# wangjunchi/LLMSeg

Measured on AMD Instinct MI355X. Metric: images/sec (1024x1024, 64-tok prompt) model_forward fwd+bwd, higher is better.
Workload: dtype bf16; 1 GPU; BASELINE.json configs[2]: synthetic 1024x1024 + random-init LLaVA-7B(Llama-7B+CLIP-L/14)/SAM-ViT-H, batch_size=2 per GPU, fwd+bwd train step (CE + align + IoP losses, LoRA r=8 dropout 0.05 on q/v + trainable embed/lm_head/text_fcs/lisa_*, frozen towers, fp32 gradient arena, AdamW step every 10 micro-steps inside the timed region, micro-step replayed from a hipGraph), 256 candidate masks, 64-token ; global_batch=2, parallelism=dp1, graph=True, valid=True

## Files before the change

### llmseg_amd/csrc/capi.cpp

```cpp
#include <hip/hip_runtime.h>
#include <stdarg.h>
#include <stdio.h>
#include <stdlib.h>
#include <algorithm>
#include <array>
#include <map>
#include <mutex>
#include <string>
#include <vector>
#include "llmseg_hip.h"

static thread_local char g_err[512] = "";

void llmseg_set_error(const char* fmt, ...) {
  va_list ap;
  va_start(ap, fmt);
  vsnprintf(g_err, sizeof(g_err), fmt, ap);
  va_end(ap);
}

extern "C" const char* llmseg_last_error(void) { return g_err; }

#include <atomic>
static std::atomic<long> g_launches{0};
// ... 53 lines not shown
  g_prof_on = on != 0;
  return LLMSEG_OK;
}

extern "C" const char* llmseg_prof_dominant_kernel(void) { return g_dom_name; }
extern "C" double llmseg_prof_dominant_bytes(void) { return g_dom_bytes; }
extern "C" int llmseg_prof_dominant_info(int64_t* out4) {
  if (!out4) return LLMSEG_EINVAL;
  for (int i = 0; i < 4; ++i) out4[i] = g_dom_info[i];
  return LLMSEG_OK;
}

extern "C" int llmseg_prof_collect(double* total_ms, double* total_flops, int64_t* launches, double* dom_ms, double* dom_flops, int64_t* dom_launches) {
  std::lock_guard<std::mutex> lk(g_mu);
  double ms = 0, fl = 0;
  std::map<long, std::array<double, 4>> by_class;
  std::map<std::array<long, 4>, std::array<double, 3>> by_shape;
  std::map<long, std::array<int64_t, 3>> split_by_class;
  for (auto& r : g_recs) {
    (void)hipEventSynchronize(r.b);
    float t = 0;
    (void)hipEventElapsedTime(&t, r.a, r.b);
    ms += t;
    fl += r.flops;
    auto& c = by_class[((r.tag[3] % 10000) / 1000) * 2 + (r.tag[3] & 1)];
    c[0] += t; c[1] += r.flops; c[2] += 1;
    {
      const long S = r.tag[3] / 10000;
      auto& sp = split_by_class[((r.tag[3] % 10000) / 1000) * 2 + (r.tag[3] & 1)];
      if (S > 1) { sp[0] += 1; sp[1] += S; }
    }
    c[3] += 2.0 * ((double)r.tag[0] * r.tag[2] + (double)r.tag[1] * r.tag[2] + (double)r.tag[0] * r.tag[1]);
    auto& e = by_shape[{r.tag[0], r.tag[1], r.tag[2], r.tag[3]}];
    e[0] += t; e[1] += r.flops; e[2] += 1;
    g_pool.push_back(r);
  }
  if (getenv("LLMSEG_PROF_TABLE")) {
    std::vector<std::pair<double, std::array<long, 4>>> order;
    for (auto& kv : by_shape) order.push_back({-kv.second[0], kv.first});
    std::sort(order.begin(), order.end());
    fprintf(stderr, "%8s %8s %8s %6s %8s %10s %9s %6s\n", "M", "N", "K", "var", "calls", "total_ms", "TFLOP/s", "%time");
    const size_t top = (size_t)std::max(40, atoi(getenv("LLMSEG_PROF_TABLE")));
    for (size_t i = 0; i < order.size() && i < top; ++i) {
      auto& e = by_shape[order[i].second];
      fprintf(stderr, "%8ld %8ld %8ld %6ld %8.0f %10.2f %9.1f %6.1f\n", order[i].second[0], order[i].second[1], order[i].second[2], order[i].second[3],
              e[2], e[0], e[1] / (e[0] * 1e-3) / 1e12, 100.0 * e[0] / ms);
    }
  }
  if (total_ms) *total_ms = ms;
  if (total_flops) *total_flops = fl;
  if (launches) *launches = (int64_t)g_recs.size();
  long dom = -1;
  for (auto& kv : by_class) if (dom < 0 || kv.second[0] > by_class[dom][0]) dom = kv.first;
  static const char* names[] = {"gemm_bf16_tn_kernel<*, ...> (register staging, 128x128)", "?", "gemm_bf16_tn_glds_kernel<*, 2, 1>", "gemm_skinny_kernel<M>", "?", "?", "?", "gemm_bf16_tn_pp2_kernel<*, false>",
                                "gemm_bf16_tn_pp_kernel<*, false, 4>", "gemm_bf16_tn_pp_kernel<*, false, 2>"};
  if (dom >= 0) {
    const long v = dom / 2;
    std::string nm = (v >= 0 && v < 10) ? names[v] : "?";
    const size_t star = nm.find('*');
    if (star != std::string::npos) nm.replace(star, 1, (dom & 1) ? "true" : "false");
    snprintf(g_dom_name, sizeof(g_dom_name), "%s", nm.c_str());
  } else g_dom_name[0] = 0;
  if (dom_ms) *dom_ms = dom >= 0 ? by_class[dom][0] : 0;
  if (dom_flops) *dom_flops = dom >= 0 ? by_class[dom][1] : 0;
  if (dom_launches) *dom_launches = dom >= 0 ? (int64_t)by_class[dom][2] : 0;
  g_dom_bytes = dom >= 0 ? by_class[dom][3] : 0;
  if (dom >= 0) {
    const auto& sp = split_by_class[dom];
    g_dom_info[0] = (int64_t)by_class[dom][2]; g_dom_info[1] = sp[0]; g_dom_info[2] = sp[1]; g_dom_info[3] = (int64_t)by_class[dom][2] + sp[0];
  } else g_dom_info[0] = g_dom_info[1] = g_dom_info[2] = g_dom_info[3] = 0;
  g_recs.clear();
  return LLMSEG_OK;
}
```

### llmseg_amd/csrc/gemm.hip

```cpp
#include <algorithm>
#include <cstdlib>
#include "common.h"
#include "llmseg_hip.h"

namespace {

constexpr int BN = 128, BK = 64, NT = 256;
constexpr int GROUP_M = 8;

struct GemmP {
  const bf16_t* A; const bf16_t* W; void* C;
  const bf16_t* bias; const bf16_t* gamma; const bf16_t* res;
  int M, N, K;
  long lda, ldw, ldc, ldr, sA, sW, sC, sA2, sW2, sC2;
  int batch1;
  float alpha;
  int act;
  int tiles_m, tiles_n;
  int c_vec, r_vec, b_vec;
  const bf16_t* A2; const bf16_t* W2; long lda2, ldw2;
  int group_m;
  int skew;
  int kt_total;
  int accum;
// ... 897 lines not shown
  const int nt = nt_main + (EXT ? 1 : 0);
  auto ext_a = [&](int h, int i) {
    const int ra = PP_AROW0(h, i) + (lane >> 3);
    return p.A2 + (long)min(m0 + ra, p.M - 1) * p.lda2 + (((lane & 7) ^ ((ra >> 1) & 7)) << 3);
  };
  auto ext_w = [&](int h, int i) {
    const int rw = PP_WROW0(h, i) + (lane >> 3);
    return p.W2 + (long)min(n0 + rw, p.N - 1) * p.ldw2 + (((lane & 7) ^ ((rw >> 1) & 7)) << 3);
  };

  f32x4_t acc[4][2 * MI];
#pragma unroll
  for (int nb = 0; nb < 4; ++nb)
#pragma unroll
    for (int mb = 0; mb < 2 * MI; ++mb) acc[nb][mb] = f32x4_t{0.f, 0.f, 0.f, 0.f};
  bf16x8_t af[MI][2], wf0[2][2], wf1[2][2];
  const int frow = lane & 15, fq = lane >> 4;
  const int wrow0 = FX == FX_ROPE ? (wn >> 1) * 128 + (wn & 1) * 32 : FX == FX_SWIGLU ? wn * 32 : wn * 64;
  const int wrow1 = wrow0 + (FX == FX_ROPE ? 64 : FX == FX_SWIGLU ? 128 : 32);

  char* cur = smem;
  char* nxt = smem + BUF;
  char* nn = smem + 2 * BUF;
  if (EXT) { PP_ISSUE_AX(0, cur); PP_ISSUE_WX(0, cur); PP_ISSUE_WX(1, cur); PP_ISSUE_AX(1, cur); }
  else { PP_ISSUE_A(0, 0, cur); PP_ISSUE_W(0, 0, cur); PP_ISSUE_W(1, 0, cur); PP_ISSUE_A(1, 0, cur); }
  PP_ISSUE_A(0, 1, nxt); PP_ISSUE_W(0, 1, nxt); PP_ISSUE_W(1, 1, nxt); PP_ISSUE_A(1, 1, nxt);
  PP_VMI(6);
  __builtin_amdgcn_s_barrier();
  if (wm == 1) __builtin_amdgcn_s_barrier();
  __builtin_amdgcn_sched_barrier(0);

#define PP2_READ_A P16_READ_W(wf0, 0, cur); P16_READ_W(wf1, 1, cur); P16_READ_A(0, cur)
#define PP2_MMA_A P16_MMA(wf0, 0, 0); P16_MMA(wf1, 2, 0)
#define PP2_MMA_B P16_MMA(wf1, 2, MI); P16_MMA(wf0, 0, MI)
  int t = 0;
  for (; t < nt - 2; ++t) {
    PP_PHASE(PP2_READ_A, PP_ISSUE_A(0, t + 2, nn); PP_ISSUE_W(0, t + 2, nn), PP_NOP, PP2_MMA_A);
    PP_PHASE(P16_READ_A(MI, cur), PP_ISSUE_W(1, t + 2, nn); PP_ISSUE_A(1, t + 2, nn), PP_VMI(6), PP2_MMA_B);
    char* const tmp = cur; cur = nxt; nxt = nn; nn = tmp;
  }
  PP_PHASE(PP2_READ_A, PP_NOP, PP_NOP, PP2_MMA_A);
  PP_PHASE(P16_READ_A(MI, cur), PP_NOP, PP_VM_0, PP2_MMA_B);
  cur = nxt;
  PP_PHASE(PP2_READ_A, PP_NOP, PP_NOP, PP2_MMA_A);
  PP_PHASE(P16_READ_A(MI, cur), PP_NOP, PP_NOP, PP2_MMA_B);
#undef PP2_READ_A
#undef PP2_MMA_A
#undef PP2_MMA_B
  if (wm == 0) __builtin_amdgcn_s_barrier();
  if constexpr (FX != FX_NONE) epilogue_fx<MI, FX>(p, Acc16<MI>{acc}, smem, wave, m0, n0, wm, wn, lane);
  else epilogue_lds<OUT_F32, MI>(p, Acc16<MI>{acc}, smem, wave, m0, n0, wm, wn, lane, bz);
}

template <int MT, int AT, bool SK = false>
__global__ __launch_bounds__(256) void gemm_skinny_kernel(GemmP p, int out_f32) {
  constexpr int KS = MT >= 4 ? 1 : 2;
  constexpr int STEP = KS * 512;
  constexpr int ADV = SK ? 4 * STEP : STEP;
  constexpr int XB = AT == 2 ? MT : 1;
  const int lane = threadIdx.x & 63, wave = threadIdx.x >> 6;
  const int n0 = SK ? blockIdx.x * 4 : (blockIdx.x * 4 + wave) * 4;
  if (n0 >= p.N) return;
  const bf16_t* wr[4];
#pragma unroll
  for (int r = 0; r < 4; ++r) wr[r] = p.W + (long)min(n0 + r, p.N - 1) * p.ldw;
  float acc[4][MT];
#pragma unroll
  for (int r = 0; r < 4; ++r)
#pragma unroll
    for (int m = 0; m < MT; ++m) acc[r][m] = 0.f;
  const int K = p.K;
  auto loadw = [&](uint4 (&w)[KS][4], int k) {
#pragma unroll
    for (int t = 0; t < KS; ++t)
#pragma unroll
      for (int r = 0; r < 4; ++r) w[t][r] = *reinterpret_cast<const uint4*>(wr[r] + min(k + t * 512, K - 8));
  };
  auto loadx = [&](uint4 (&xa)[KS][MT], uint4 (&xb)[KS][XB], int k) {
#pragma unroll
    for (int t = 0; t < KS; ++t) {
      const int kk = k + t * 512, kc = min(kk, K - 8);
      const bool ok = kk < K;
#pragma unroll
      for (int m = 0; m < MT; ++m) {
        const bf16_t* ar = p.A + (long)min(m, p.M - 1) * p.lda;
        const uint4 v = *reinterpret_cast<const uint4*>(ar + kc);
        xa[t][m] = make_uint4(ok ? v.x : 0u, ok ? v.y : 0u, ok ? v.z : 0u, ok ? v.w : 0u);
        if constexpr (AT == 2) xb[t][m] = *reinterpret_cast<const uint4*>(ar + K + kc);
      }
      if constexpr (AT == 1) xb[t][0] = *reinterpret_cast<const uint4*>(p.a_norm_w + kc);
    }
  };
  float rstd[MT];
  auto xform = [&](const uint4& a, const uint4& b, int m) -> uint4 {
    if constexpr (AT == 0) return a;
    float f[8], g[8], o[8];
    unpack8(a, f);
    unpack8(b, g);
    if constexpr (AT == 1) {
      const float r = rstd[m];
      const uint4 xn = make_uint4(pack2bf(f[0] * r, f[1] * r), pack2bf(f[2] * r, f[3] * r), pack2bf(f[4] * r, f[5] * r), pack2bf(f[6] * r, f[7] * r));
      unpack8(xn, f);
#pragma unroll
      for (int e = 0; e < 8; ++e) o[e] = g[e] * f[e];
    } else {
#pragma unroll
// ... 211 lines not shown
__global__ __launch_bounds__(256) void splitk_reduce_delta_kernel(GemmP p, const float* __restrict__ slab, int S, const bf16_t* __restrict__ O, long ldo,
                                                                 float* __restrict__ delta, int heads, int T) {
  const long m = blockIdx.x;
  const int nch = p.N >> 3;
  const long slab_sz = (long)p.M * p.N;
  const long b = m / T, q = m - b * T;
#pragma unroll
  for (int i = 0; i < CPT; ++i) {
    const int c = threadIdx.x + 256 * i;
    if (c < nch) {
      const int n = c * 8;
      const float* sp = slab + m * p.N + n;
      float4 a0 = *reinterpret_cast<const float4*>(sp), a1 = *reinterpret_cast<const float4*>(sp + 4);
      for (int s2 = 1; s2 < S; ++s2) {
        const float4 b0 = *reinterpret_cast<const float4*>(sp + s2 * slab_sz), b1 = *reinterpret_cast<const float4*>(sp + s2 * slab_sz + 4);
        a0.x += b0.x; a0.y += b0.y; a0.z += b0.z; a0.w += b0.w;
        a1.x += b1.x; a1.y += b1.y; a1.z += b1.z; a1.w += b1.w;
      }
      const float v[8] = {a0.x * p.alpha, a0.y * p.alpha, a0.z * p.alpha, a0.w * p.alpha, a1.x * p.alpha, a1.y * p.alpha, a1.z * p.alpha, a1.w * p.alpha};
      const uint4 g = pack8(v);
      *reinterpret_cast<uint4*>(reinterpret_cast<bf16_t*>(p.C) + m * p.ldc + n) = g;
      float of[8], df[8];
      unpack8(*reinterpret_cast<const uint4*>(O + m * ldo + n), of);
      unpack8(g, df);
      float part = 0.f;
#pragma unroll
      for (int e = 0; e < 8; ++e) part = fmaf(of[e], df[e], part);
#pragma unroll
      for (int mm = 8; mm >= 1; mm >>= 1) part += __shfl_xor(part, mm, 64);
      if ((c & 15) == 0) delta[(b * heads + (c >> 4)) * T + q] = part;
    }
  }
}

struct NormReq { const bf16_t* w; bf16_t* out; long ldn; float eps; bool active, done; };
static thread_local NormReq g_norm_req = {nullptr, nullptr, 0, 0.f, false, false};
struct NbReq { const llmseg_gemm_args* a; void* out; bool active, done; };
static thread_local NbReq g_nb_req = {nullptr, nullptr, false, false};
struct DlReq { const llmseg_gemm_args* a; bool active, done; };
static thread_local DlReq g_dl_req = {nullptr, false, false};

template <bool OUT_F32, int MI, int NBUF>
void launch_glds(const GemmP& p, dim3 grid, hipStream_t s) {
  LL_LAUNCH_KERNEL((gemm_bf16_tn_glds_kernel<OUT_F32, MI, NBUF>), grid, dim3(NT), 0, s, p);
}

}

void llmseg_prof_begin(hipStream_t s);
void llmseg_prof_end(hipStream_t s, double flops);
void llmseg_prof_tag(long a, long b, long c, long d);

static int g_gemm_variant = 5, g_gemm_skew = 13, g_gemm_split = 0, g_gemm_pp2 = getenv("LLMSEG_GEMM_PP2") ? atoi(getenv("LLMSEG_GEMM_PP2")) : 1;
static const int g_gemm_rsplit = getenv("LLMSEG_GEMM_NO_RSPLIT") ? 0 : 1;
static int num_cus() {
  static int n = [] { int dev = 0, v = 0; (void)hipGetDevice(&dev); (void)hipDeviceGetAttribute(&v, hipDeviceAttributeMultiprocessorCount, dev); return v > 0 ? v : 256; }();
  return n;
}
extern "C" int llmseg_gemm_set_variant(int v) {
  g_gemm_variant = v & 15;
  if ((v >> 4) & 15) g_gemm_skew = ((v >> 4) & 15) - 1;
  g_gemm_split = (v >> 8) & 31;
  g_gemm_pp2 = (v >> 13) & 3 ? ((v >> 13) & 3) - 1 : g_gemm_pp2;
  return LLMSEG_OK;
}

namespace {
struct GemmPlan { int variant, split; double us; };
inline double pp_cost(long M, long N, int nt, int mi, int S, long ncu, bool f32out) {
  const long tiles = ((M + 64 * mi - 1) / (64 * mi)) * ((N + 255) / 256);
  const long rounds = (tiles * S + ncu - 1) / ncu;
  const int q = (nt + S - 1) / S;
  const double it = mi == 4 ? 1.7 : 1.0, fix = (mi == 4 ? 7.0 : 4.5) + ((S > 1 || f32out) ? 1.0 : 0.0);
  double eff_rounds = (double)rounds;
  if (S == 1) {
    const long full = tiles / ncu, rem = tiles - full * ncu;
    eff_rounds = (double)full + (rem ? 0.5 + 0.5 * (double)rem / (double)ncu : 0.0);
  }
  double us = eff_rounds * (q * it + fix);
  if (S > 1) us += 2.5 + ((double)(S + 1) * M * N * 4.0) / 4.0e6;
  return us;
}
inline double glds_cost(long M, long N, int nt, long ncu) {
  const long tiles = ((M + 127) / 128) * ((N + 127) / 128);
  const long full = tiles / (4 * ncu), rem = tiles - full * 4 * ncu;
  double us = (double)full * (nt * 2.4 + 4.0);
  if (rem > 0) { const double w = (double)((rem + ncu - 1) / ncu); us += nt * std::max(1.3, 0.6 * w) + 4.0; }
  return us;
}
inline bool split_ok(int nt, int S) {
  if (S <= 1) return S == 1;
  const int q = (nt + S - 1) / S;
  return q >= 2 && nt - (S - 1) * q >= 2;
}
}

static int gemm_dispatch(const llmseg_gemm_args* a, void* stream, int force_variant);

extern "C" int llmseg_norm(const void* x, const void* w, const void* b, void* y, int64_t rows, int64_t cols, int64_t ldx, int64_t ldy, float eps, int rms,
                           const int32_t* row_map, void* stream);

extern "C" int llmseg_rope(void* x, const float* cos, const float* sin, int64_t rows, int64_t T, int32_t heads, int32_t head_dim, int64_t ld, void* stream);
extern "C" int llmseg_swiglu(const void* gu, void* out, int64_t rows, int64_t I, int64_t ldgu, int64_t ldo, void* stream);
extern "C" __attribute__((visibility("hidden"))) int llmseg_swiglu_bwd_ld(const void* gu, const void* dout, void* dgu, int64_t rows, int64_t I, int64_t ld_dout, void* stream);

static thread_local bool g_fx_done = false;
static const bool g_fx_off = getenv("LLMSEG_GEMM_NO_FX") != nullptr;

static int gemm_fx(const llmseg_gemm_args* a, void* stream) {
  LL_CHECK(a->fx >= 1 && a->fx <= 3, "gemm: unknown fx %d", a->fx);
  LL_CHECK(!a->out_f32 && a->batch <= 1 && a->batch2 <= 1 && a->alpha == 1.f && !a->bias && !a->gamma && !a->residual && a->act == LLMSEG_ACT_NONE && !a->norm_out &&
               !a->trans_a && !a->trans_w && !a->accumulate, "gemm: fx needs a plain bf16 product (batch 1, alpha 1, no bias / activation / gamma / residual / norm_out)");
  if (a->fx == LLMSEG_FX_ROPE) {
    LL_CHECK(a->fx_cos && a->fx_sin && a->fx_T > 0 && a->fx_cols > 0 && (a->fx_cols % 128) == 0 && a->fx_cols <= a->N && (a->ldc & 3) == 0 &&
                 ((((uintptr_t)a->fx_cos) | ((uintptr_t)a->fx_sin)) & 15) == 0 && (((uintptr_t)a->C) & 7) == 0,
             "gemm: fx rope needs fp32 [fx_T][64] tables (16-byte aligned), fx_cols a multiple of 128 (heads of width 128) and <= N");
  } else if (a->fx == LLMSEG_FX_SWIGLU) {
    LL_CHECK(a->fx_out && (a->N & 15) == 0 && (a->fx_ld & 7) == 0 && a->fx_ld >= a->N / 2 && (a->ldc & 7) == 0 && !a->A2 && ((((uintptr_t)a->fx_out) | ((uintptr_t)a->C)) & 15) == 0,
             "gemm: fx swiglu needs N = 2 I with I %% 8 == 0, fx_out bf16 [M][fx_ld >= I], 16-byte aligned rows, no extension operands");
  } else {
    LL_CHECK(a->fx_in && (a->N & 7) == 0 && (a->fx_ld & 7) == 0 && a->fx_ld >= 2 * a->N && a->ldc >= 2 * a->N && (a->ldc & 7) == 0 && !a->A2 &&
                 ((((uintptr_t)a->fx_in) | ((uintptr_t)a->C)) & 15) == 0,
             "gemm: fx swiglu_bwd needs N = I, fx_in = gate|up bf16 [M][fx_ld >= 2 I], C = d(gate|up) [M][ldc >= 2 I], 16-byte aligned rows");
  }
  g_fx_done = false;
  llmseg_gemm_args g = *a;
// ... 74 lines not shown
  if (a && a->struct_size == sizeof(*a) && a->dl_o) return gemm_dl(a, stream);
  if (!(a && a->struct_size == sizeof(*a) && a->norm_out)) return gemm_dispatch(a, stream, -1);
  LL_CHECK(a->norm_w && !a->out_f32 && a->batch <= 1 && a->batch2 <= 1 && (a->N & 7) == 0 && (a->ldn & 7) == 0 && a->ldn >= a->N && (a->ldc & 7) == 0 &&
               ((((uintptr_t)a->norm_w) | ((uintptr_t)a->norm_out) | ((uintptr_t)a->C)) & 15) == 0 && !a->accumulate,
           "gemm: norm_out needs norm_w, bf16 output, batch 1, N, ldc and ldn multiples of 8, 16-byte aligned pointers");
  g_norm_req = NormReq{(const bf16_t*)a->norm_w, (bf16_t*)a->norm_out, (long)a->ldn, a->norm_eps, true, false};
  const int rc = gemm_dispatch(a, stream, -1);
  const bool done = g_norm_req.done;
  g_norm_req.active = false;
  if (rc != LLMSEG_OK || done) return rc;
  return llmseg_norm(a->C, a->norm_w, nullptr, a->norm_out, a->M, a->N, a->ldc, a->ldn, a->norm_eps, 1, nullptr, stream);
}

static int gemm_dispatch(const llmseg_gemm_args* a, void* stream, int force_variant) {
  LL_CHECK(a && a->struct_size == sizeof(*a), "%s: ABI mismatch: caller's struct_size %u != %zu (bind against include/llmseg_hip.h version %d)",
           "gemm", a ? a->struct_size : 0u, sizeof(*a), LLMSEG_ABI_VERSION);
  LL_CHECK(a && a->A && a->W && a->C, "gemm: null pointer");
  LL_CHECK(a->M > 0 && a->N > 0 && a->K > 0, "gemm: bad shape M=%ld N=%ld K=%ld", (long)a->M, (long)a->N, (long)a->K);
  const bool ta = a->trans_a != 0, tw = a->trans_w != 0;
  LL_CHECK((a->lda & 7) == 0 && (a->ldw & 7) == 0, "gemm: lda/ldw must be multiples of 8 (lda=%ld ldw=%ld)", (long)a->lda, (long)a->ldw);
  const long k8 = (a->K + 7) & ~7L;
  LL_CHECK((ta || (a->K & 7) == 0 || a->lda >= k8) && (tw || (a->K & 7) == 0 || a->ldw >= k8),
           "gemm: K=%ld is not a multiple of 8 and the K-contiguous operand is not padded", (long)a->K);
  LL_CHECK((!ta || a->lda >= a->M) && (!tw || a->ldw >= a->N), "gemm: transposed operand needs ld >= rows");
  LL_CHECK((((uintptr_t)a->A) & 15) == 0 && (((uintptr_t)a->W) & 15) == 0, "gemm: A/W must be 16-byte aligned");
  LL_CHECK(((a->strideA | a->strideW | a->strideA2 | a->strideW2) & 7) == 0, "gemm: batch strides of A/W must be multiples of 8");
  LL_CHECK(!a->accumulate || a->out_f32, "gemm: accumulate needs fp32 output");
  const int esz = a->out_f32 ? 4 : 2;
  GemmP p;
  p.A = (const bf16_t*)a->A; p.W = (const bf16_t*)a->W; p.C = a->C;
  p.bias = (const bf16_t*)a->bias; p.gamma = (const bf16_t*)a->gamma; p.res = (const bf16_t*)a->residual;
  p.M = (int)a->M; p.N = (int)a->N; p.K = (int)a->K;
  p.lda = a->lda; p.ldw = a->ldw; p.ldc = a->ldc; p.ldr = a->residual ? a->ldr : 0;
  const long batch1 = a->batch > 0 ? a->batch : 1, batch2 = a->batch2 > 0 ? a->batch2 : 1;
  const long batch = batch1 * batch2;
  p.batch1 = (int)batch1;
  p.sA = a->strideA; p.sW = a->strideW; p.sC = a->strideC;
  p.sA2 = a->strideA2; p.sW2 = a->strideW2; p.sC2 = a->strideC2;
  p.alpha = a->alpha; p.act = a->act;
  p.kt_total = 0; p.k_split_total = 0; p.accum = a->accumulate ? 1 : 0;
  p.fx = 0; p.fx_T = a->fx_T; p.fx_cols = (int)a->fx_cols; p.fx_I = a->fx == LLMSEG_FX_SWIGLU ? (int)(a->N / 2) : (int)a->N;
  p.fx_cos = a->fx_cos; p.fx_sin = a->fx_sin; p.fx_out = (bf16_t*)a->fx_out; p.fx_in = (const bf16_t*)a->fx_in; p.fx_ld = a->fx_ld;
  { static const int abl = getenv("LLMSEG_LW_ABLATE") ? atoi(getenv("LLMSEG_LW_ABLATE")) : 0; p.ablate = abl; }
  p.c_vec = ((((uintptr_t)a->C) % (4 * esz)) == 0 && (a->ldc & 3) == 0 && ((a->strideC | a->strideC2) & 3) == 0) ? 1 : 0;
  p.r_vec = (p.res && (((uintptr_t)p.res) & 7) == 0 && (p.ldr & 3) == 0 && ((a->strideC | a->strideC2) & 3) == 0) ? 1 : 0;
  p.b_vec = ((p.bias == nullptr || (((uintptr_t)p.bias) & 7) == 0) && (p.gamma == nullptr || (((uintptr_t)p.gamma) & 7) == 0)) ? 1 : 0;

  p.skew = g_gemm_skew;
  p.A2 = (const bf16_t*)a->A2; p.W2 = (const bf16_t*)a->W2; p.lda2 = a->lda2; p.ldw2 = a->ldw2;
  static const int group_m_env = getenv("LLMSEG_GEMM_GROUP_M") ? atoi(getenv("LLMSEG_GEMM_GROUP_M")) : 0;
  const int nt = p.K / BK;
  const long ncu = num_cus();
  int variant = (p.K % BK == 0 && !ta && !tw) ? (force_variant >= 0 ? force_variant : g_gemm_variant) : 0;
  if (variant != 0 && variant != 2 && variant != 3 && variant != 8 && variant != 9) variant = 5;
  if ((variant == 8 || variant == 9) && nt < (a->A2 ? 1 : 2)) variant = 2;
  const bool can_split = batch == 1 && (p.N & 3) == 0 && (p.ldc & 3) == 0 && a->workspace != nullptr &&
                         (((uintptr_t)a->workspace) & 15) == 0 && (!p.res || (p.ldr & 3) == 0);
  auto ws_fits = [&](int S) { return (double)(S + (a->A2 ? 1 : 0)) * p.M * p.N * 4.0 <= (double)a->workspace_bytes; };
  int split = 1;
  if (variant == 5) {
    GemmPlan best{2, 1, glds_cost(p.M, p.N, nt, ncu) * (double)batch};
    if (nt >= (a->A2 ? 1 : 2)) {
      for (int mi = 4; mi >= 2; mi -= 2) {
        for (int S = 1; S <= 16; ++S) {
          if (S > 1 && (!can_split || !split_ok(nt, S) || !ws_fits(S))) continue;
          if (S > 1 && ((p.M + 64 * mi - 1) / (64 * mi)) * ((p.N + 255) / 256) * S > ncu) break;
          const double us = pp_cost(p.M, p.N, nt, mi, S, ncu, a->out_f32 != 0) * (double)batch;
          if (us < best.us * 0.97 || (us < best.us && S == 1)) best = GemmPlan{mi == 4 ? 8 : 9, S, us};
        }
      }
    }
    static const int g4_env = getenv("LLMSEG_GEMM_G4") ? atoi(getenv("LLMSEG_GEMM_G4")) : 0;
    if (g4_env && !a->A2 && nt >= 2) {
      const long t128 = (long)((p.M + 127) / 128) * ((p.N + 127) / 128) * batch;
      if (t128 <= ncu) {
        const double us = nt * 0.55 + 4.0;
        if (us < best.us) best = GemmPlan{3, 1, us};
      }
    }
    variant = best.variant; split = best.split;
  } else if (variant == 8 || variant == 9) {
    split = (g_gemm_split > 1 && force_variant < 0) ? g_gemm_split : 1;
    if (split > 1) LL_CHECK(can_split && split_ok(nt, split) && ws_fits(split), "gemm: forced split-K %d not possible for this call", split);
  }
  if (p.A2) {
    LL_CHECK(p.W2 && batch == 1 && !ta && !tw && (p.lda2 & 7) == 0 && (p.ldw2 & 7) == 0 && p.lda2 >= 64 && p.ldw2 >= 64 &&
                 (((uintptr_t)p.A2 | (uintptr_t)p.W2) & 15) == 0, "gemm: bad extension operands (A2 [M][64], W2 [N][64], 16-byte aligned rows)");
    LL_CHECK(!a->out_f32, "gemm: extension operands need bf16 output");
    if ((variant == 8 || variant == 9) && split > 1) {
      llmseg_gemm_args g2 = *a;
      g2.A = a->A2; g2.W = a->W2; g2.lda = a->lda2; g2.ldw = a->ldw2; g2.K = 64; g2.A2 = g2.W2 = nullptr;
      g2.bias = g2.gamma = g2.residual = nullptr; g2.alpha = 1.f; g2.act = LLMSEG_ACT_NONE; g2.out_f32 = 1; g2.accumulate = 0;
      g2.C = (float*)a->workspace + (long)split * p.M * p.N; g2.ldc = p.N; g2.workspace = nullptr; g2.workspace_bytes = 0;
      g2.norm_w = nullptr; g2.norm_out = nullptr;
      const bool pend = g_norm_req.active;
      g_norm_req.active = false;
      const int rc = llmseg_gemm_bf16(&g2, stream);
      g_norm_req.active = pend;
      if (rc != LLMSEG_OK) return rc;
    } else if (variant != 8 && variant != 9) {
      LL_CHECK(a->act == LLMSEG_ACT_NONE && !a->gamma, "gemm: extension operands on this shape need a linear epilogue");
      llmseg_gemm_args g1 = *a, g2 = *a;
      g1.A2 = g1.W2 = nullptr;
      g1.norm_w = g2.norm_w = nullptr; g1.norm_out = g2.norm_out = nullptr;
      g_norm_req.active = false;
      int rc = llmseg_gemm_bf16(&g1, stream);
      if (rc != LLMSEG_OK) return rc;
      g2.A = a->A2; g2.W = a->W2; g2.lda = a->lda2; g2.ldw = a->ldw2; g2.K = 64; g2.bias = nullptr; g2.residual = a->C; g2.ldr = a->ldc;
      g2.A2 = g2.W2 = nullptr;
      return llmseg_gemm_bf16(&g2, stream);
    }
  }
  p.a_norm_w = (const bf16_t*)a->a_norm_w; p.a_norm_eps = a->a_norm_eps; p.a_swiglu = a->a_swiglu;
  const bool a_xform = p.a_norm_w || p.a_swiglu;
  LL_CHECK(!a_xform || (p.M <= 8 && !ta && !tw && batch == 1 && !p.A2 && (p.K & 7) == 0 && !(p.a_norm_w && p.a_swiglu) &&
                        (!p.a_norm_w || (((uintptr_t)p.a_norm_w) & 15) == 0) && (!p.a_swiglu || p.lda >= 2 * p.K)),
           "gemm: A-row transforms (a_norm_w / a_swiglu) are decode-step fusions of the M <= 8 route");
  if (p.M <= 8 && !ta && !tw && batch == 1 && !p.A2 && (p.K & 7) == 0 && (g_gemm_variant == 5 || a_xform)) {
    hipStream_t s = (hipStream_t)stream;
    llmseg_prof_begin(s);
    llmseg_prof_tag(p.M, p.N, p.K, 3000 + (p.res ? 20 : 0) + p.act * 2 + (a->out_f32 ? 1 : 0));
    static const int sk_env = getenv("LLMSEG_SKINNY_SK") ? atoi(getenv("LLMSEG_SKINNY_SK")) : 1;
    const bool sk = sk_env == 2 ? p.K >= 2048 : (sk_env && p.N <= 8192 && p.K >= 2048);
    const dim3 grid((unsigned)(sk ? (p.N + 3) / 4 : (p.N + 15) / 16));
    const int of = a->out_f32 ? 1 : 0;
#define LL_SKINNY_(AT, SKV)                                                                                   \
    do {                                                                                                      \
      if (p.M == 1) LL_LAUNCH_KERNEL((gemm_skinny_kernel<1, AT, SKV>), grid, dim3(256), 0, s, p, of);      \
      else if (p.M == 2) LL_LAUNCH_KERNEL((gemm_skinny_kernel<2, AT, SKV>), grid, dim3(256), 0, s, p, of); \
      else if (p.M <= 4) LL_LAUNCH_KERNEL((gemm_skinny_kernel<4, AT, SKV>), grid, dim3(256), 0, s, p, of); \
      else LL_LAUNCH_KERNEL((gemm_skinny_kernel<8, AT, SKV>), grid, dim3(256), 0, s, p, of);               \
    } while (0)
#define LL_SKINNY(AT) do { if (sk) LL_SKINNY_(AT, true); else LL_SKINNY_(AT, false); } while (0)
    if (p.a_norm_w) LL_SKINNY(1); else if (p.a_swiglu) LL_SKINNY(2); else LL_SKINNY(0);
#undef LL_SKINNY_
#undef LL_SKINNY
    llmseg_prof_end(s, 2.0 * (double)a->M * (double)a->N * (double)a->K);
    LL_LAUNCH_CHECK("gemm_skinny");
    return LLMSEG_OK;
  }
  const bool pp = variant == 8 || variant == 9;
  const int bm = variant == 8 ? 256 : 128, bn = pp ? 256 : BN;
  p.tiles_m = (p.M + bm - 1) / bm; p.tiles_n = (p.N + bn - 1) / bn;
  static const bool old_walk = getenv("LLMSEG_GEMM_OLD_WALK") != nullptr;
  p.group_m = group_m_env > 0 ? group_m_env : (p.tiles_m <= 32 ? ((p.tiles_n > 16 && p.tiles_m > 8 && !old_walk) ? 8 : p.tiles_m) : 4);
  hipStream_t s = (hipStream_t)stream;
  llmseg_prof_begin(s);
  llmseg_prof_tag(p.M, p.N, p.K, (variant == 9 && g_gemm_pp2 ? 7 : variant) * 1000 + (ta ? 200 : 0) + (tw ? 100 : 0) + (p.res ? 20 : 0) + p.act * 2 + (a->out_f32 ? 1 : 0) + 40 * (batch > 1) +
                  10000 * (split > 1 ? split : 0));
  const bool f = a->out_f32 != 0;
  if (variant == 0 && batch2 == 1 && (p.N & 3) == 0 && (p.ldc & 3) == 0 && a->workspace != nullptr && (((uintptr_t)a->workspace) & 15) == 0 &&
      (!p.res || ((p.ldr & 3) == 0 && batch == 1)) && ((p.sC & 3) == 0 || batch == 1) && g_gemm_rsplit) {
    const long tiles = (long)p.tiles_m * p.tiles_n * batch;
    const int ntr = (p.K + BK - 1) / BK;
    int S = (tiles * 4 <= ncu && ntr >= 8) ? (int)std::min<long>({(long)ncu / std::max<long>(tiles, 1), (long)ntr / 2, 32L}) : 1;
    while (S > 1 && (double)S * batch * p.M * p.N * 4.0 > (double)a->workspace_bytes) --S;
    if (S > 1) {
      const int q = (ntr + S - 1) / S;
      S = (ntr + q - 1) / q;
    }
    if (S > 1) {
      const int q = (ntr + S - 1) / S;
      static const bool log_it = getenv("LLMSEG_RSPLIT_LOG") != nullptr;
      if (log_it) fprintf(stderr, "rsplit M=%d N=%d K=%d ta=%d tw=%d S=%d q=%d f32=%d acc=%d res=%d bias=%d act=%d lda=%ld ldw=%ld ldc=%ld batch=%ld alpha=%g\n", p.M, p.N, p.K,
                          (int)ta, (int)tw, S, q, (int)f, p.accum, p.res != nullptr, p.bias != nullptr, p.act, p.lda, p.ldw, p.ldc, batch, p.alpha);
      GemmP ps = p;
      ps.K = q * BK; ps.k_split_total = p.K; ps.batch1 = S;
      ps.sA = ta ? (long)q * BK * p.lda : (long)q * BK; ps.sW = tw ? (long)q * BK * p.ldw : (long)q * BK;
      ps.sA2 = p.sA; ps.sW2 = p.sW;
      ps.C = a->workspace; ps.ldc = p.N; ps.sC = (long)p.M * p.N; ps.sC2 = (long)S * p.M * p.N;
      ps.bias = ps.gamma = ps.res = nullptr; ps.ldr = 0; ps.alpha = 1.f; ps.act = LLMSEG_ACT_NONE; ps.accum = 0;
      ps.c_vec = 1; ps.r_vec = 0; ps.b_vec = 1;
      const dim3 grid(p.tiles_m * p.tiles_n, (unsigned)(S * batch));
      const int key = (ta ? 2 : 0) | (tw ? 1 : 0);
      switch (key) {
        case 0: LL_LAUNCH_KERNEL((gemm_bf16_tn_kernel<true, false, false>), grid, dim3(NT), 0, s, ps); break;
        case 1: LL_LAUNCH_KERNEL((gemm_bf16_tn_kernel<true, false, true>), grid, dim3(NT), 0, s, ps); break;
        case 2: LL_LAUNCH_KERNEL((gemm_bf16_tn_kernel<true, true, false>), grid, dim3(NT), 0, s, ps); break;
        default: LL_LAUNCH_KERNEL((gemm_bf16_tn_kernel<true, true, true>), grid, dim3(NT), 0, s, ps); break;
      }
      const long total4 = (long)p.M * (p.N >> 2);
      const unsigned rg = (unsigned)std::min<long>((total4 + 255) / 256, 4096);
      LL_LAUNCH_KERNEL(splitk_reduce_kernel, dim3(rg, (unsigned)batch), dim3(256), 0, s, p, (const float*)a->workspace, S, f ? 1 : 0);
      llmseg_prof_end(s, 2.0 * (double)a->M * (double)a->N * (double)a->K * (double)batch);
      LL_LAUNCH_CHECK("gemm_bf16_tn (K-sliced)");
      return LLMSEG_OK;
    }
  }
  if (pp && split > 1) {
    GemmP ps = p;
    const int q = (nt + split - 1) / split;
    ps.K = q * BK; ps.kt_total = nt; ps.batch1 = split;
    ps.sA = ps.sW = (long)q * BK; ps.sA2 = ps.sW2 = ps.sC2 = 0;
    ps.C = a->workspace; ps.ldc = p.N; ps.sC = (long)p.M * p.N;
    ps.bias = ps.gamma = ps.res = nullptr; ps.ldr = 0; ps.alpha = 1.f; ps.act = LLMSEG_ACT_NONE; ps.accum = 0;
    ps.c_vec = 1; ps.r_vec = 0; ps.b_vec = 1; ps.A2 = ps.W2 = nullptr;
    dim3 grid(p.tiles_m * p.tiles_n, (unsigned)split);
    if (variant == 8) LL_LAUNCH_KERNEL((gemm_bf16_tn_pp_kernel<true, false, 4>), grid, dim3(NTB), 0, s, ps);
    else if (g_gemm_pp2 == 2) LL_LAUNCH_KERNEL((gemm_bf16_tn_lw_kernel<true>), grid, dim3(NTL), 0, s, ps);
    else if (g_gemm_pp2) LL_LAUNCH_KERNEL((gemm_bf16_tn_pp2_kernel<true, false>), grid, dim3(NTB), 0, s, ps);
    else LL_LAUNCH_KERNEL((gemm_bf16_tn_pp_kernel<true, false, 2>), grid, dim3(NTB), 0, s, ps);
    const long total4 = (long)p.M * (p.N >> 2);
    const unsigned rg = (unsigned)std::min<long>((total4 + 255) / 256, 4096);
    static const long wg_max_rows = getenv("LLMSEG_NORM_WG_MAX") ? atol(getenv("LLMSEG_NORM_WG_MAX")) : 2048;
    static const bool no_fuse = getenv("LLMSEG_GEMM_NO_NORM_FUSE") != nullptr;
    const bool fuse_norm = g_norm_req.active && !no_fuse && !f && p.alpha == 1.f && !p.bias && !p.gamma && p.act == LLMSEG_ACT_NONE && p.M >= 64 && p.M < wg_max_rows &&
                           p.N >= 2048 && p.N <= 8192 && (p.N & 7) == 0 && (p.ldc & 7) == 0 && (!p.res || (p.ldr & 7) == 0) && (g_norm_req.ldn & 7) == 0 &&
                           ((((uintptr_t)p.C) | ((uintptr_t)p.res) | ((uintptr_t)g_norm_req.w) | ((uintptr_t)g_norm_req.out)) & 15) == 0;
    const bool fuse_nb = g_nb_req.active && !f && p.alpha == 1.f && !p.bias && !p.gamma && !p.res && p.act == LLMSEG_ACT_NONE && p.M >= 64 && p.N >= 2048 && p.N <= 8192 &&
                         (p.N & 7) == 0;
    const bool fuse_dl = g_dl_req.active && !f && !p.bias && !p.gamma && !p.res && p.act == LLMSEG_ACT_NONE && p.N <= 8192 && (p.N & 127) == 0 && (p.ldc & 7) == 0;
    if (fuse_dl) {
      const llmseg_gemm_args* q = g_dl_req.a;
      const int S2 = split + (p.A2 ? 1 : 0);
      const int cpt = ((p.N >> 3) + 255) / 256;
#define LL_RDL(C) LL_LAUNCH_KERNEL(splitk_reduce_delta_kernel<C>, dim3((unsigned)p.M), dim3(256), 0, s, p, (const float*)a->workspace, S2, (const bf16_t*)q->dl_o, \
                                   (long)q->dl_ldo, q->dl_out, (int)q->dl_heads, (int)q->dl_T)
      if (cpt <= 1) LL_RDL(1); else if (cpt <= 2) LL_RDL(2); else LL_RDL(4);
#undef LL_RDL
      g_dl_req.done = true;
    } else if (fuse_nb) {
      const llmseg_gemm_args* q = g_nb_req.a;
      const int rc = llmseg_reduce_lora_normbwd((const float*)a->workspace, split + (p.A2 ? 1 : 0), p.M, p.N, q->nb_x, q->nb_w, g_nb_req.out, q->nb_eps, q->nb_rms, q->nb_dres,
                                                (void*)q->nb_lora_t, q->nb_lora_ldt, q->nb_lora_w0, q->nb_lora_w1, q->nb_lora_alpha, (const llmseg_dropout*)q->nb_lora_drop,
                                                q->nb_lora_part, q->nb_lora_S, q->nb_lora_scale, q->nb_lora_zero, stream);
      if (rc != LLMSEG_OK) return rc;
      g_nb_req.done = true;
    } else if (fuse_norm) {
      const int S2 = split + (p.A2 ? 1 : 0);
      const int cpt = ((p.N >> 3) + 255) / 256;
      if (cpt <= 1) LL_LAUNCH_KERNEL(splitk_reduce_rmsnorm_kernel<1>, dim3((unsigned)p.M), dim3(256), 0, s, p, (const float*)a->workspace, S2, g_norm_req.w, g_norm_req.eps, g_norm_req.out, g_norm_req.ldn);
      else if (cpt <= 2) LL_LAUNCH_KERNEL(splitk_reduce_rmsnorm_kernel<2>, dim3((unsigned)p.M), dim3(256), 0, s, p, (const float*)a->workspace, S2, g_norm_req.w, g_norm_req.eps, g_norm_req.out, g_norm_req.ldn);
      else LL_LAUNCH_KERNEL(splitk_reduce_rmsnorm_kernel<4>, dim3((unsigned)p.M), dim3(256), 0, s, p, (const float*)a->workspace, S2, g_norm_req.w, g_norm_req.eps, g_norm_req.out, g_norm_req.ldn);
      g_norm_req.done = true;
    } else
    LL_LAUNCH_KERNEL(splitk_reduce_kernel, dim3(rg), dim3(256), 0, s, p, (const float*)a->workspace, split + (p.A2 ? 1 : 0), f ? 1 : 0);
  } else {
    dim3 grid(p.tiles_m * p.tiles_n, (unsigned)batch);
    switch (variant) {
      case 2: f ? launch_glds<true, 2, 1>(p, grid, s) : launch_glds<false, 2, 1>(p, grid, s); break;
      case 3:
        if (f) LL_LAUNCH_KERNEL((gemm_bf16_tn_g4_kernel<true>), grid, dim3(NT), 0, s, p);
        else LL_LAUNCH_KERNEL((gemm_bf16_tn_g4_kernel<false>), grid, dim3(NT), 0, s, p);
        break;
      case 8: {
        const bool fx_ok8 = a->fx && !g_fx_off && !f && batch == 1 &&
                            (a->fx == LLMSEG_FX_ROPE ? (p.N % 256) == 0 && p.A2 != nullptr
                             : a->fx == LLMSEG_FX_SWIGLU ? (p.fx_I % 128) == 0 : (p.N % 64) == 0);
        if (fx_ok8) {
          GemmP q = p;
          q.fx = a->fx;
// ... 61 lines not shown
```

Baseline: 49.99 images/s.

## Add 160x256 K-sliced GEMM tile kernel and include it in planner

Adds a new GEMM kernel with a 160-row by 256-column tile that writes fp32 partials for split-K and is reduced by the existing reduce path. The cost model gains a 160-row option, and the planner now considers it for split-K counts of two or more when there is no fused epilogue or residual. The aim is better CU fill and less tile-quantization waste for M shapes that fit poorly into 128- or 256-row tiles. In exchange it adds an uneven wave-to-row mapping for the A loads and relies on a hand-set per-K-tile cost constant that may choose it poorly.

Result: faster. 51.26 images/s (median of 6 runs) (+2.5%).

```diff
diff --git a/llmseg_amd/csrc/capi.cpp b/llmseg_amd/csrc/capi.cpp
--- a/llmseg_amd/csrc/capi.cpp
+++ b/llmseg_amd/csrc/capi.cpp
@@ -129,7 +129,7 @@
   if (launches) *launches = (int64_t)g_recs.size();
   long dom = -1;
   for (auto& kv : by_class) if (dom < 0 || kv.second[0] > by_class[dom][0]) dom = kv.first;
-  static const char* names[] = {"gemm_bf16_tn_kernel<*, ...> (register staging, 128x128)", "?", "gemm_bf16_tn_glds_kernel<*, 2, 1>", "gemm_skinny_kernel<M>", "?", "?", "?", "gemm_bf16_tn_pp2_kernel<*, false>",
+  static const char* names[] = {"gemm_bf16_tn_kernel<*, ...> (register staging, 128x128)", "?", "gemm_bf16_tn_glds_kernel<*, 2, 1>", "gemm_skinny_kernel<M>", "?", "?", "gemm_bf16_tn_t160_kernel (K-sliced)", "gemm_bf16_tn_pp2_kernel<*, false>",
                                 "gemm_bf16_tn_pp_kernel<*, false, 4>", "gemm_bf16_tn_pp_kernel<*, false, 2>"};
   if (dom >= 0) {
     const long v = dom / 2;
diff --git a/llmseg_amd/csrc/gemm.hip b/llmseg_amd/csrc/gemm.hip
--- a/llmseg_amd/csrc/gemm.hip
+++ b/llmseg_amd/csrc/gemm.hip
@@ -973,6 +973,151 @@
   else epilogue_lds<OUT_F32, MI>(p, Acc16<MI>{acc}, smem, wave, m0, n0, wm, wn, lane, bz);
 }
 
+constexpr int T160_BM = 160;
+#define T160_BL(rs, dst, voff, tt) __builtin_amdgcn_raw_ptr_buffer_load_lds(rs, (lds_ptr_t)(dst), 16, voff, (int)((tt) * (BK * 2)), 0, 0)
+#define T160_ISSUE_A0(tt, base) T160_BL(rsrc_a, (base) + a_lds0, a_off0, tt)
+#define T160_ISSUE_A1(tt, base)                                       \
+  do {                                                                \
+    T160_BL(rsrc_a, (base) + a_lds1[0], a_off1[0], tt);               \
+    if (two) T160_BL(rsrc_a, (base) + a_lds1[1], a_off1[1], tt);      \
+  } while (0)
+#define T160_ISSUE_W(h, tt, base)                                     \
+  do {                                                                \
+    T160_BL(rsrc_w, (base) + w_lds[h][0], w_off[h][0], tt);           \
+    T160_BL(rsrc_w, (base) + w_lds[h][1], w_off[h][1], tt);           \
+  } while (0)
+#define T160_VM_TILE do { if (two) PP_VMI(7); else PP_VMI(6); } while (0)
+#define T160_READ_A(cnt, mb0, base)                                                                                           \
+  _Pragma("unroll") for (int mb = 0; mb < (cnt); ++mb) _Pragma("unroll") for (int ks = 0; ks < 2; ++ks)                     \
+      af[mb][ks] = *reinterpret_cast<const bf16x8_t*>((base) + lds_off(wm * 80 + ((mb0) + mb) * 16 + frow, ks * 4 + fq))
+#define T160_MMA(wfx, nb0, cnt, mb0)                                                                                          \
+  _Pragma("unroll") for (int ks = 0; ks < 2; ++ks) _Pragma("unroll") for (int nb = 0; nb < 2; ++nb)                         \
+      _Pragma("unroll") for (int mb = 0; mb < (cnt); ++mb)                                                                    \
+          acc[(nb0) + nb][(mb0) + mb] = __builtin_amdgcn_mfma_f32_16x16x32_bf16(wfx[nb][ks], af[mb][ks], acc[(nb0) + nb][(mb0) + mb], 0, 0, 0)
+
+__global__ __launch_bounds__(NTB, 2) void gemm_bf16_tn_t160_kernel(GemmP p) {
+  constexpr int BMB = T160_BM, BNB = 256;
+  constexpr int A_BYTES = BMB * BK * 2, W_BYTES = BNB * BK * 2, BUF = A_BYTES + W_BYTES;
+  __shared__ __attribute__((aligned(16))) char smem[3 * BUF];
+  int bid = blockIdx.x;
+  const int nwg = p.tiles_m * p.tiles_n;
+  {
+    const int q = nwg >> 3, r = nwg & 7, xcd = bid & 7;
+    const int len = q + (xcd < r ? 1 : 0);
+    const int idx = ((bid >> 3) + xcd * p.skew) % len;
+    bid = (xcd < r ? xcd * (q + 1) : r * (q + 1) + (xcd - r) * q) + idx;
+  }
+  const int per_group = p.group_m * p.tiles_n;
+  const int first_m = (bid / per_group) * p.group_m;
+  const int gsz = min(p.tiles_m - first_m, p.group_m);
+  const int m0 = (first_m + (bid % per_group) % gsz) * BMB;
+  const int n0 = ((bid % per_group) / gsz) * BNB;
+
+  const int tid = threadIdx.x, lane = tid & 63;
+  const int wave = __builtin_amdgcn_readfirstlane(tid >> 6);
+  const int wm = wave >> 2, wn = wave & 3;
+  const bool two = wn < 2;
+  const long b1 = blockIdx.y;
+  const bf16_t* __restrict__ Ag = p.A + b1 * p.sA;
+  const bf16_t* __restrict__ Wg = p.W + b1 * p.sW;
+  const __amdgpu_buffer_rsrc_t rsrc_a = __builtin_amdgcn_make_buffer_rsrc(const_cast<bf16_t*>(Ag + (long)m0 * p.lda), 0, 0x7fffffff, 0x00020000);
+  const __amdgpu_buffer_rsrc_t rsrc_w = __builtin_amdgcn_make_buffer_rsrc(const_cast<bf16_t*>(Wg + (long)n0 * p.ldw), 0, 0x7fffffff, 0x00020000);
+  auto a_src = [&](int ra0) { const int ra = ra0 + (lane >> 3); return (int)(((long)min(ra, p.M - 1 - m0) * p.lda + (((lane & 7) ^ ((ra >> 1) & 7)) << 3)) * 2); };
+  const int ra_a0 = wm * 80 + wn * 8;
+  const int j1 = 8 + 2 * wm + (wn & 1);
+  const int ra_a1[2] = {(wave / 6) * 80 + 32 + (wave % 6) * 8, (j1 / 6) * 80 + 32 + (j1 % 6) * 8};
+  const int a_lds0 = ra_a0 * 128, a_off0 = a_src(ra_a0);
+  const int a_lds1[2] = {ra_a1[0] * 128, ra_a1[1] * 128};
+  const int a_off1[2] = {a_src(ra_a1[0]), a_src(ra_a1[1])};
+  int w_off[2][2], w_lds[2][2];
+#pragma unroll
+  for (int h = 0; h < 2; ++h) {
+#pragma unroll
+    for (int i = 0; i < 2; ++i) {
+      const int rw0 = PP_WROW0(h, i), rw = rw0 + (lane >> 3);
+      w_lds[h][i] = A_BYTES + rw0 * 128;
+      w_off[h][i] = (int)(((long)min(rw, p.N - 1 - n0) * p.ldw + (((lane & 7) ^ ((rw >> 1) & 7)) << 3)) * 2);
+    }
+  }
+  int nt = p.K / BK;
+  nt = min(nt, p.kt_total - (int)b1 * nt);
+
+  f32x4_t acc[4][5];
+#pragma unroll
+  for (int nb = 0; nb < 4; ++nb)
+#pragma unroll
+    for (int mb = 0; mb < 5; ++mb) acc[nb][mb] = f32x4_t{0.f, 0.f, 0.f, 0.f};
+  bf16x8_t af[3][2], wf0[2][2], wf1[2][2];
+  const int frow = lane & 15, fq = lane >> 4;
+  const int wrow0 = wn * 64, wrow1 = wrow0 + 32;
+
+  char* cur = smem;
+  char* nxt = smem + BUF;
+  char* nn = smem + 2 * BUF;
+  T160_ISSUE_A0(0, cur); T160_ISSUE_W(0, 0, cur); T160_ISSUE_W(1, 0, cur); T160_ISSUE_A1(0, cur);
+  T160_ISSUE_A0(1, nxt); T160_ISSUE_W(0, 1, nxt); T160_ISSUE_W(1, 1, nxt); T160_ISSUE_A1(1, nxt);
+  T160_VM_TILE;
+  __builtin_amdgcn_s_barrier();
+  if (wm == 1) __builtin_amdgcn_s_barrier();
+  __builtin_amdgcn_sched_barrier(0);
+
+#define T160_RD_A P16_READ_W(wf0, 0, cur); P16_READ_W(wf1, 1, cur); T160_READ_A(2, 0, cur)
+#define T160_RD_B T160_READ_A(3, 2, cur)
+#define T160_MMA_A T160_MMA(wf0, 0, 2, 0); T160_MMA(wf1, 2, 2, 0)
+#define T160_MMA_B T160_MMA(wf1, 2, 3, 2); T160_MMA(wf0, 0, 3, 2)
+  int t = 0;
+  for (; t < nt - 2; ++t) {
+    PP_PHASE(T160_RD_A, T160_ISSUE_A0(t + 2, nn); T160_ISSUE_W(0, t + 2, nn), PP_NOP, T160_MMA_A);
+    PP_PHASE(T160_RD_B, T160_ISSUE_W(1, t + 2, nn); T160_ISSUE_A1(t + 2, nn), T160_VM_TILE, T160_MMA_B);
+    char* const tmp = cur; cur = nxt; nxt = nn; nn = tmp;
+  }
+  PP_PHASE(T160_RD_A, PP_NOP, PP_NOP, T160_MMA_A);
+  PP_PHASE(T160_RD_B, PP_NOP, PP_VMI(0), T160_MMA_B);
+  cur = nxt;
+  PP_PHASE(T160_RD_A, PP_NOP, PP_NOP, T160_MMA_A);
+  PP_PHASE(T160_RD_B, PP_NOP, PP_NOP, T160_MMA_B);
+#undef T160_RD_A
+#undef T160_RD_B
+#undef T160_MMA_A
+#undef T160_MMA_B
+  if (wm == 0) __builtin_amdgcn_s_barrier();
+
+  float* slab = reinterpret_cast<float*>(smem) + wave * (32 * 64);
+  const int r15 = lane & 15, q4 = lane >> 4;
+  const int c = lane & 15, rsub = lane >> 4;
+  const int n = n0 + wn * 64 + c * 4;
+  const int mw = m0 + wm * 80;
+  float* cbase = reinterpret_cast<float*>(p.C) + b1 * p.sC;
+#pragma unroll
+  for (int i = 0; i < 3; ++i) {
+    const int nh = i < 2 ? 2 : 1;
+#pragma unroll
+    for (int h = 0; h < nh; ++h)
+#pragma unroll
+      for (int nb = 0; nb < 4; ++nb) {
+        const int row = h * 16 + r15, chunk = nb * 4 + q4;
+        *reinterpret_cast<float4*>(slab + row * 64 + ((chunk ^ (row & 15)) << 2)) =
+            make_float4(acc[nb][2 * i + h][0], acc[nb][2 * i + h][1], acc[nb][2 * i + h][2], acc[nb][2 * i + h][3]);
+      }
+#pragma unroll
+    for (int it = 0; it < 4 * nh; ++it) {
+      const int row = it * 4 + rsub;
+      const float4 a4 = *reinterpret_cast<const float4*>(slab + row * 64 + ((c ^ (row & 15)) << 2));
+      const int m = mw + i * 32 + row;
+      if (m >= p.M || n >= p.N) continue;
+      *reinterpret_cast<float4*>(cbase + (long)m * p.ldc + n) =
+          make_float4(fmaf(a4.x, p.alpha, 0.f), fmaf(a4.y, p.alpha, 0.f), fmaf(a4.z, p.alpha, 0.f), fmaf(a4.w, p.alpha, 0.f));
+    }
+  }
+}
+#undef T160_BL
+#undef T160_ISSUE_A0
+#undef T160_ISSUE_A1
+#undef T160_ISSUE_W
+#undef T160_VM_TILE
+#undef T160_READ_A
+#undef T160_MMA
+
 template <int MT, int AT, bool SK = false>
 __global__ __launch_bounds__(256) void gemm_skinny_kernel(GemmP p, int out_f32) {
   constexpr int KS = MT >= 4 ? 1 : 2;
@@ -1290,6 +1435,7 @@
 void llmseg_prof_tag(long a, long b, long c, long d);
 
 static int g_gemm_variant = 5, g_gemm_skew = 13, g_gemm_split = 0, g_gemm_pp2 = getenv("LLMSEG_GEMM_PP2") ? atoi(getenv("LLMSEG_GEMM_PP2")) : 1;
+static const bool g_gemm_t160 = getenv("LLMSEG_GEMM_NO_T160") == nullptr;
 static const int g_gemm_rsplit = getenv("LLMSEG_GEMM_NO_RSPLIT") ? 0 : 1;
 static int num_cus() {
   static int n = [] { int dev = 0, v = 0; (void)hipGetDevice(&dev); (void)hipDeviceGetAttribute(&v, hipDeviceAttributeMultiprocessorCount, dev); return v > 0 ? v : 256; }();
@@ -1305,11 +1451,12 @@
 
 namespace {
 struct GemmPlan { int variant, split; double us; };
-inline double pp_cost(long M, long N, int nt, int mi, int S, long ncu, bool f32out) {
-  const long tiles = ((M + 64 * mi - 1) / (64 * mi)) * ((N + 255) / 256);
+constexpr double T160_KT_US = 1.13;
+inline double pp_cost(long M, long N, int nt, int bm, int S, long ncu, bool f32out) {
+  const long tiles = ((M + bm - 1) / bm) * ((N + 255) / 256);
   const long rounds = (tiles * S + ncu - 1) / ncu;
   const int q = (nt + S - 1) / S;
-  const double it = mi == 4 ? 1.7 : 1.0, fix = (mi == 4 ? 7.0 : 4.5) + ((S > 1 || f32out) ? 1.0 : 0.0);
+  const double it = bm == 256 ? 1.7 : bm == 160 ? T160_KT_US : 1.0, fix = (bm == 256 ? 7.0 : 4.5) + ((S > 1 || f32out) ? 1.0 : 0.0);
   double eff_rounds = (double)rounds;
   if (S == 1) {
     const long full = tiles / ncu, rem = tiles - full * ncu;
@@ -1490,8 +1637,9 @@
   const int nt = p.K / BK;
   const long ncu = num_cus();
   int variant = (p.K % BK == 0 && !ta && !tw) ? (force_variant >= 0 ? force_variant : g_gemm_variant) : 0;
-  if (variant != 0 && variant != 2 && variant != 3 && variant != 8 && variant != 9) variant = 5;
+  if (variant != 0 && variant != 2 && variant != 3 && variant != 8 && variant != 9 && variant != 10) variant = 5;
   if ((variant == 8 || variant == 9) && nt < (a->A2 ? 1 : 2)) variant = 2;
+  if (variant == 10 && nt < 2) variant = 2;
   const bool can_split = batch == 1 && (p.N & 3) == 0 && (p.ldc & 3) == 0 && a->workspace != nullptr &&
                          (((uintptr_t)a->workspace) & 15) == 0 && (!p.res || (p.ldr & 3) == 0);
   auto ws_fits = [&](int S) { return (double)(S + (a->A2 ? 1 : 0)) * p.M * p.N * 4.0 <= (double)a->workspace_bytes; };
@@ -1499,12 +1647,14 @@
   if (variant == 5) {
     GemmPlan best{2, 1, glds_cost(p.M, p.N, nt, ncu) * (double)batch};
     if (nt >= (a->A2 ? 1 : 2)) {
-      for (int mi = 4; mi >= 2; mi -= 2) {
-        for (int S = 1; S <= 16; ++S) {
+      const bool t160 = g_gemm_t160 && !a->fx && !a->residual;
+      for (const int bm : {256, 128, 160}) {
+        if (bm == 160 && !t160) continue;
+        for (int S = bm == 160 ? 2 : 1; S <= 16; ++S) {
           if (S > 1 && (!can_split || !split_ok(nt, S) || !ws_fits(S))) continue;
-          if (S > 1 && ((p.M + 64 * mi - 1) / (64 * mi)) * ((p.N + 255) / 256) * S > ncu) break;
-          const double us = pp_cost(p.M, p.N, nt, mi, S, ncu, a->out_f32 != 0) * (double)batch;
-          if (us < best.us * 0.97 || (us < best.us && S == 1)) best = GemmPlan{mi == 4 ? 8 : 9, S, us};
+          if (S > 1 && ((p.M + bm - 1) / bm) * ((p.N + 255) / 256) * S > ncu) break;
+          const double us = pp_cost(p.M, p.N, nt, bm, S, ncu, a->out_f32 != 0) * (double)batch;
+          if (us < best.us * 0.97 || (us < best.us && S == 1)) best = GemmPlan{bm == 256 ? 8 : bm == 160 ? 10 : 9, S, us};
         }
       }
     }
@@ -1520,12 +1670,15 @@
   } else if (variant == 8 || variant == 9) {
     split = (g_gemm_split > 1 && force_variant < 0) ? g_gemm_split : 1;
     if (split > 1) LL_CHECK(can_split && split_ok(nt, split) && ws_fits(split), "gemm: forced split-K %d not possible for this call", split);
+  } else if (variant == 10) {
+    split = g_gemm_split;
+    LL_CHECK(split > 1 && can_split && split_ok(nt, split) && ws_fits(split), "gemm: variant 10 (160 x 256, K-sliced) needs a forced split-K count >= 2 that is possible for this call (got %d)", split);
   }
   if (p.A2) {
     LL_CHECK(p.W2 && batch == 1 && !ta && !tw && (p.lda2 & 7) == 0 && (p.ldw2 & 7) == 0 && p.lda2 >= 64 && p.ldw2 >= 64 &&
                  (((uintptr_t)p.A2 | (uintptr_t)p.W2) & 15) == 0, "gemm: bad extension operands (A2 [M][64], W2 [N][64], 16-byte aligned rows)");
     LL_CHECK(!a->out_f32, "gemm: extension operands need bf16 output");
-    if ((variant == 8 || variant == 9) && split > 1) {
+    if ((variant == 8 || variant == 9 || variant == 10) && split > 1) {
       llmseg_gemm_args g2 = *a;
       g2.A = a->A2; g2.W = a->W2; g2.lda = a->lda2; g2.ldw = a->ldw2; g2.K = 64; g2.A2 = g2.W2 = nullptr;
       g2.bias = g2.gamma = g2.residual = nullptr; g2.alpha = 1.f; g2.act = LLMSEG_ACT_NONE; g2.out_f32 = 1; g2.accumulate = 0;
@@ -1536,7 +1689,7 @@
       const int rc = llmseg_gemm_bf16(&g2, stream);
       g_norm_req.active = pend;
       if (rc != LLMSEG_OK) return rc;
-    } else if (variant != 8 && variant != 9) {
+    } else if (variant != 8 && variant != 9 && variant != 10) {
       LL_CHECK(a->act == LLMSEG_ACT_NONE && !a->gamma, "gemm: extension operands on this shape need a linear epilogue");
       llmseg_gemm_args g1 = *a, g2 = *a;
       g1.A2 = g1.W2 = nullptr;
@@ -1577,14 +1730,14 @@
     LL_LAUNCH_CHECK("gemm_skinny");
     return LLMSEG_OK;
   }
-  const bool pp = variant == 8 || variant == 9;
-  const int bm = variant == 8 ? 256 : 128, bn = pp ? 256 : BN;
+  const bool pp = variant == 8 || variant == 9 || variant == 10;
+  const int bm = variant == 8 ? 256 : variant == 10 ? T160_BM : 128, bn = pp ? 256 : BN;
   p.tiles_m = (p.M + bm - 1) / bm; p.tiles_n = (p.N + bn - 1) / bn;
   static const bool old_walk = getenv("LLMSEG_GEMM_OLD_WALK") != nullptr;
   p.group_m = group_m_env > 0 ? group_m_env : (p.tiles_m <= 32 ? ((p.tiles_n > 16 && p.tiles_m > 8 && !old_walk) ? 8 : p.tiles_m) : 4);
   hipStream_t s = (hipStream_t)stream;
   llmseg_prof_begin(s);
-  llmseg_prof_tag(p.M, p.N, p.K, (variant == 9 && g_gemm_pp2 ? 7 : variant) * 1000 + (ta ? 200 : 0) + (tw ? 100 : 0) + (p.res ? 20 : 0) + p.act * 2 + (a->out_f32 ? 1 : 0) + 40 * (batch > 1) +
+  llmseg_prof_tag(p.M, p.N, p.K, (variant == 9 && g_gemm_pp2 ? 7 : variant == 10 ? 6 : variant) * 1000 + (ta ? 200 : 0) + (tw ? 100 : 0) + (p.res ? 20 : 0) + p.act * 2 + (a->out_f32 ? 1 : 0) + 40 * (batch > 1) +
                   10000 * (split > 1 ? split : 0));
   const bool f = a->out_f32 != 0;
   if (variant == 0 && batch2 == 1 && (p.N & 3) == 0 && (p.ldc & 3) == 0 && a->workspace != nullptr && (((uintptr_t)a->workspace) & 15) == 0 &&
@@ -1635,6 +1788,7 @@
     ps.c_vec = 1; ps.r_vec = 0; ps.b_vec = 1; ps.A2 = ps.W2 = nullptr;
     dim3 grid(p.tiles_m * p.tiles_n, (unsigned)split);
     if (variant == 8) LL_LAUNCH_KERNEL((gemm_bf16_tn_pp_kernel<true, false, 4>), grid, dim3(NTB), 0, s, ps);
+    else if (variant == 10) LL_LAUNCH_KERNEL(gemm_bf16_tn_t160_kernel, grid, dim3(NTB), 0, s, ps);
     else if (g_gemm_pp2 == 2) LL_LAUNCH_KERNEL((gemm_bf16_tn_lw_kernel<true>), grid, dim3(NTL), 0, s, ps);
     else if (g_gemm_pp2) LL_LAUNCH_KERNEL((gemm_bf16_tn_pp2_kernel<true, false>), grid, dim3(NTB), 0, s, ps);
     else LL_LAUNCH_KERNEL((gemm_bf16_tn_pp_kernel<true, false, 2>), grid, dim3(NTB), 0, s, ps);
```
